# SKIRT/SKIRT9

Measured on AMD Instinct MI355X. Metric: photon packets/s (whole node), 10^6-cell octree, higher is better.
Workload: dtype f64

## Files before the change

skirt9_amd/csrc/pmc_cycle.inc:

```

    enum Event : int { EV_NONE = 0, EV_LAUNCH = 1, EV_CYCLE_DONE = 2, EV_TASK = 5, EV_DEAD = 6 };


    template<bool EMISSION = false>
    __device__ __forceinline__ int nextObserver(const DevScene& S, int slot, double rx, double ry, double rz, int g)
    {
        const SlotArrays& A = S.slots;
        while (g < S.num_instruments)
        {
            bool need = false;
            int j = g;
            do
            {
                const DevInstrument& I = S.inst[j];
                const bool seen = (I.include_sed && insideAperture(I, rx, ry, rz)) || (I.include_ifu && pixelOnDetector(I, rx, ry, rz) >= 0);
                if (seen && (EMISSION ? A.obsEll[(int64_t)j * A.num_slots + slot] : S.mono ? S.inst[j].mono_ell : A.ell[(int64_t)j * A.num_slots + slot]) >= 0)
                    need = true;
                ++j;
            } while (j < S.num_instruments && S.inst[j].same_observer);
            if (need) return g;
            g = j;
        }
        return g;
    }

    constexpr int PEEL_SORT_TILE = 2048;
    __device__ __forceinline__ uint32_t peelTile(const PeelSortArgs& ps, const DevInstrument& I, double x, double y, double z)
    {
        x -= ps.centre[0], y -= ps.centre[1], z -= ps.centre[2];
        const double xpp = -I.sinphi * x + I.cosphi * y;
        const double ypp = -I.cosphi * I.costheta * x - I.sinphi * I.costheta * y + I.sintheta * z;
        int tx = (int)(xpp * ps.scale + 0.5 * PMC_PEEL_TILES), ty = (int)(ypp * ps.scale + 0.5 * PMC_PEEL_TILES);
        tx = tx < 0 ? 0 : tx >= PMC_PEEL_TILES ? PMC_PEEL_TILES - 1 : tx;
        ty = ty < 0 ? 0 : ty >= PMC_PEEL_TILES ? PMC_PEEL_TILES - 1 : ty;
        return (uint32_t)(ty * PMC_PEEL_TILES + tx);
    }
#ifndef PMC_PROP_KEY_CONES
#define PMC_PROP_KEY_CONES 1
#endif
#ifndef PMC_PROP_KEY_BLOCKS
#define PMC_PROP_KEY_BLOCKS 1
#endif
    __device__ __forceinline__ uint32_t propSortKey(const DevScene& S, double x, double y, double z, double kx, double ky, double kz)
    {
#if PMC_PROP_KEY_CONES
        const uint32_t oct = S.grid_kind == PMC_GRID_VORONOI ? (uint32_t)(voroCone(kx, ky, kz) >> 2)
                                                             : (kx < 0. ? 1u : 0u) | (ky < 0. ? 2u : 0u) | (kz < 0. ? 4u : 0u);
#else
        const uint32_t oct = (kx < 0. ? 1u : 0u) | (ky < 0. ? 2u : 0u) | (kz < 0. ? 4u : 0u);
#endif
        constexpr int B = PMC_PROP_KEY_BLOCKS;
        int ix = (int)((x - S.gx0) / (S.gx1 - S.gx0) * B), iy = (int)((y - S.gy0) / (S.gy1 - S.gy0) * B), iz = (int)((z - S.gz0) / (S.gz1 - S.gz0) * B);
        ix = ix < 0 ? 0 : ix >= B ? B - 1 : ix;
        iy = iy < 0 ? 0 : iy >= B ? B - 1 : iy;
        iz = iz < 0 ? 0 : iz >= B ? B - 1 : iz;
        return oct * (uint32_t)(B * B * B) + (uint32_t)((iz * B + iy) * B + ix);
    }
    template<int GRID>
    __device__ __forceinline__ bool prepareWalk(const DevScene& S, const GridLds& G, Counters& cnt, int slot, int record, int mode,
                                                double rx, double ry, double rz, double kx, double ky, double kz, double target,
                                                double sext, int& hint, PeelRec* sortedOut = nullptr, bool deferScan = false)
    {
        const SlotArrays& A = S.slots;
        const TaskArrays& K = S.tasks;
        const int64_t t = (int64_t)record * A.num_slots + slot;
        Walk w;
        w.rx = rx, w.ry = ry, w.rz = rz;
        setDirection(w, kx, ky, kz);
        if (mode == MODE_PASS1) target = INFINITY;
        const bool zeroPeel = mode == MODE_PEEL && target == -INFINITY;
        if (mode == MODE_PEEL && !zeroPeel) target = nextAfterToward(target, true);
        cnt.paths += 1;
        int located;
        const bool ok = startWalk<GRID>(S, G, w, (GRID == GRID_CART) ? -1 : hint, located, GRID == GRID_VORO && deferScan);
        if ((GRID == GRID_TREE || GRID == GRID_BIN) && located >= 0) hint = located;
        if (zeroPeel || !ok)
        {
            if (record == 0)
                A.mint[slot] = -1;
            else
                A.ptau[(int64_t)(record - 1) * A.num_slots + slot] = zeroPeel ? INFINITY : 0.;
            if (GRID == GRID_TREE && sortedOut)
                reinterpret_cast<uint4*>(sortedOut)[3] = make_uint4(0u, PMC_TASK_NONE, (uint32_t)slot, 0u);
            else
                K.bits[t] = PMC_TASK_NONE;
            return false;
        }
        if (GRID == GRID_TREE && sortedOut)
        {
            const uint32_t bits = (uint32_t)mode | ((uint32_t)w.axis << 2) | (w.sgn << 4) | (w.e << 8);
            uint4* out = reinterpret_cast<uint4*>(sortedOut);
            const double2 a = make_double2(w.rx, w.ry), b = make_double2(w.rz, w.ds);
            const unsigned long long tbits = (unsigned long long)__double_as_longlong(target), P = (unsigned long long)w.P;
            out[0] = *reinterpret_cast<const uint4*>(&a);
            out[1] = *reinterpret_cast<const uint4*>(&b);
            out[2] = make_uint4((uint32_t)tbits, (uint32_t)(tbits >> 32), (uint32_t)P, (uint32_t)(P >> 32));
            out[3] = make_uint4((uint32_t)w.cell, bits, (uint32_t)slot, 0u);
            return true;
        }
        const bool moved = GRID != GRID_TREE || w.s != 0. || w.rx != rx || w.ry != ry || w.rz != rz;
        if (moved)
        {
            K.rx[t] = w.rx, K.ry[t] = w.ry, K.rz[t] = w.rz;
            if (GRID != GRID_TREE || record == 0) K.s0[t] = w.s;
        }
        if (GRID != GRID_TREE) K.kx[t] = w.kx, K.ky[t] = w.ky, K.kz[t] = w.kz;
        if (GRID == GRID_TREE) K.pidx[t] = w.P;
        K.ds[t] = w.ds;
        if (!(GRID == GRID_TREE && mode == MODE_PASS1)) K.target[t] = target;
        K.cell[t] = w.cell;
        K.bits[t] = (uint32_t)mode | ((uint32_t)w.axis << 2) | (w.sgn << 4) | ((GRID == GRID_TREE ? w.e : 0u) << 8)
                    | ((GRID == GRID_TREE && moved) ? PMC_TASK_MOVED : 0u);
        if (GRID == GRID_VORO) K.cijk[t] = w.ci;
        return true;
    }

    template<bool DIPOLE = false, bool EMISSION = false>
    __device__ __forceinline__ void announceCycle(const DevScene& S, int slot, uint64_t seed, Rng& rng, double rx, double ry, double rz, double kinx,
                                                  double kiny, double kinz, double W, double asym, int pscatt, const double* shares = nullptr,
                                                  const double* asyms = nullptr, const DevSource* emitter = nullptr)
    {
        const SlotArrays& A = S.slots;
        const int64_t NS = A.num_slots;
        uint32_t pmask = 0;
        int g = nextObserver<EMISSION>(S, slot, rx, ry, rz, 0);
        for (int i = 0; i < S.num_instruments; ++i)
        {
            if (i != g) continue;
            const DevInstrument& I = S.inst[i];
            double pW = W;
            if (pscatt != 0 && shares)
            {
                const double costheta = kinx * I.kx + kiny * I.ky + kinz * I.kz;
                double sum = 0.;
                for (int h = 0; h < S.num_media; ++h)
                    if (shares[h] > 0.)
                    {
                        const double value = phaseValue<DIPOLE>(S, h, asyms[h], costheta);
                        sum += value * shares[h];
                    }
                pW = W * sum;
            }
            else if (pscatt != 0)
                pW = W * scatteringPeelFactor<DIPOLE>(S, asym, kinx, kiny, kinz, I);
            else if (emitter)
                pW = W * angularProbability(*emitter, I.kx, I.ky, I.kz);
            A.ppW[(int64_t)i * NS + slot] = pW;
            pmask |= 1u << i;
            int j = i + 1;
            while (j < S.num_instruments && S.inst[j].same_observer) ++j;
// ... 30 lines not shown
        for (int i = 0; i <= S.num_instruments; ++i)
        {
            const bool prop = i == S.num_instruments;
            if (!prop && !((pmask >> i) & 1u))
            {
                S.tasks.bits[(int64_t)(1 + i) * NS + slot] = PMC_TASK_NONE;
                continue;
            }
            const DevInstrument& I = S.inst[prop ? 0 : i];
            double target = prop ? drawn : peelTaumax(A.ppW[(int64_t)i * NS + slot], (KIN && emission) ? A.obsLambda[(int64_t)i * NS + slot] : lambda);
            if (KIN && emission && !prop && target != -INFINITY)
            {
                const double sobs = A.obsExt[(int64_t)i * NS + slot];
                if (sobs != sext)
                {
                    if (sext == 0.) atomicAdd(S.counters + 7, 1ull);
                    target = sobs > 0. ? target * (sext / sobs) : INFINITY;
                }
            }
            PeelRec* place = nullptr;
            const bool deferScan = GRID == GRID_VORO && ps
                                   && (prop ? ((S.voro_defer_scan & 2) != 0 && ps->propIndex >= 0)
                                            : ((S.voro_defer_scan & 1) != 0 && ps->sortIndex[i] >= 0 && S.vobs_of_inst[i] >= 0));
            if (ps && !prop)
            {
                const int k = ps->sortIndex[i];
                if (k >= 0)
                {
                    const uint32_t at = atomicAdd(&cursors[(uint32_t)k * ps->numParts + peelTile(*ps, I, rx, ry, rz)], 1u);
                    if (at >= ps->cap)
                        atomicAdd(S.counters + 7, 1ull);
                    else if (GRID == GRID_TREE)
                        place = ps->out[k] + at;
                    else
                        ps->listOut[k][at] = slot;
                }
            }
            if (GRID != GRID_TREE && ps && prop && ps->propIndex >= 0)
            {
                const uint32_t at = atomicAdd(&cursors[(uint32_t)ps->propIndex * ps->numParts + propSortKey(S, rx, ry, rz, kx, ky, kz)], 1u);
                if (at >= ps->cap)
                    atomicAdd(S.counters + 7, 1ull);
                else
                    ps->listOut[ps->propIndex][at] = slot;
            }
            const bool exists = prepareWalk<GRID>(S, G, cnt, slot, prop ? 0 : 1 + i, prop ? (S.force_scattering ? MODE_PASS1 : MODE_PASS2) : MODE_PEEL,
                                                  rx, ry, rz, prop ? kx : I.kx, prop ? ky : I.ky, prop ? kz : I.kz, target, sext, hint,
                                                  place, deferScan);
            if (exists) made |= prop ? 1u : 2u << i;
        }
        return made;
    }

    template<int GRID, bool KIN = false>
    __global__ __launch_bounds__(256, PMC_CYCLE_MIN_WAVES) void cycleStartKernel(const int sceneSlot, const int slotBase, const int numSlots,
                                                                                 const int listCounter, int* const listOut,
                                                                                 const int* const listIn, const int listLen, const PeelSortArgs ps)
    {
        const DevScene& S = c_scene[sceneSlot];
        extern __shared__ double lds[];
        const int tid = threadIdx.x;
        const int lane = tid & 63;
        if (GRID == GRID_TREE) requireLdsBaseZero(lds);
        stageGrid<GRID>(S, lds, tid, blockDim.x);
        __syncthreads();
        const GridLds G = makeGridLds(S, lds);
        const SlotArrays& A = S.slots;
        Counters cnt = {0, 0, 0, 0, 0};
        const int slotEnd = slotBase + numSlots;
        const bool sparse = GRID == GRID_TREE && listIn != nullptr;
        if (ps.numObs > 0 && !sparse)
        {
            uint32_t* const cur = reinterpret_cast<uint32_t*>(reinterpret_cast<char*>(lds) + ps.ldsOffset);
            const int numLists = ps.numObs + (ps.propIndex >= 0 ? 1 : 0);
            for (int k = 0; k < numLists; ++k)
                for (uint32_t p = tid; p < ps.numParts; p += blockDim.x)
                    cur[(uint32_t)k * ps.numParts + p] = (uint32_t)ps.start[k][p] + ps.matrix[k][(size_t)blockIdx.x * ps.numParts + p];
            __syncthreads();
            const int tiles = (numSlots + PEEL_SORT_TILE - 1) / PEEL_SORT_TILE;
            for (int t = blockIdx.x; t < tiles; t += gridDim.x)
                for (int i = t * PEEL_SORT_TILE + tid; i < (t + 1) * PEEL_SORT_TILE && i < numSlots; i += blockDim.x)
                {
                    const int slot = slotBase + i;
                    const int md = A.mode[slot];
                    if (md & MODE_ALIVE) startCycleWalks<GRID, KIN>(S, G, cnt, slot, md, &ps, cur);
                }
        }
        else
        {
            const int end = sparse ? listLen : numSlots;
            for (int i0 = blockIdx.x * blockDim.x; i0 < end; i0 += gridDim.x * blockDim.x)
            {
                const int i = i0 + tid;
                const int slot = sparse ? (i < listLen ? listIn[i] : -1) : slotBase + i;
                const int md = (slot >= 0 && slot < slotEnd) ? A.mode[slot] : 0;
                if (md & MODE_ALIVE) startCycleWalks<GRID, KIN>(S, G, cnt, slot, md);
                if (GRID == GRID_TREE && listCounter >= 0)
                {
                    const unsigned long long m = __ballot((md & MODE_ALIVE) != 0);
                    if (m)
                    {
                        unsigned long long at = 0;
                        if (lane == __ffsll((long long)m) - 1) at = atomicAdd(S.counters + listCounter, (unsigned long long)__popcll(m));
                        at = __shfl(at, __ffsll((long long)m) - 1, 64);
                        if (md & MODE_ALIVE) listOut[(int)at + __popcll(m & ((1ull << lane) - 1ull))] = slot;
                    }
                }
            }
        }
        const unsigned long long v = waveSum(cnt.paths);
        if (lane == 0 && v) atomicAdd(S.counters + 1, v);
    }

    __global__ __launch_bounds__(256) void peelSortCountKernel(const int sceneSlot, const int slotBase, const int numSlots, const PeelSortArgs ps)
    {
        const DevScene& S = c_scene[sceneSlot];
        const SlotArrays& A = S.slots;
        __shared__ uint32_t h[PMC_SORT_OBS * PMC_PEEL_TILES * PMC_PEEL_TILES];
        const int tid = threadIdx.x;
        const int numLists = ps.numObs + (ps.propIndex >= 0 ? 1 : 0);
        for (uint32_t p = tid; p < (uint32_t)numLists * ps.numParts; p += blockDim.x) h[p] = 0u;
        __syncthreads();
        const int tiles = (numSlots + PEEL_SORT_TILE - 1) / PEEL_SORT_TILE;
        for (int t = blockIdx.x; t < tiles; t += gridDim.x)
            for (int i = t * PEEL_SORT_TILE + tid; i < (t + 1) * PEEL_SORT_TILE && i < numSlots; i += blockDim.x)
            {
                const int slot = slotBase + i;
                const int md = A.mode[slot];
                if (!(md & MODE_ALIVE)) continue;
                const double x = A.rx[slot], y = A.ry[slot], z = A.rz[slot];
                for (int k = 0; k < ps.numObs; ++k)
                    if (((uint32_t)md >> (8 + ps.obs[k])) & 1u) atomicAdd(&h[(uint32_t)k * ps.numParts + peelTile(ps, S.inst[ps.obs[k]], x, y, z)], 1u);
                if (ps.propIndex >= 0)
                    atomicAdd(&h[(uint32_t)ps.propIndex * ps.numParts + propSortKey(S, x, y, z, A.kx[slot], A.ky[slot], A.kz[slot])], 1u);
            }
        __syncthreads();
        for (int k = 0; k < numLists; ++k)
            for (uint32_t p = tid; p < ps.numParts; p += blockDim.x) ps.matrix[k][(size_t)blockIdx.x * ps.numParts + p] = h[(uint32_t)k * ps.numParts + p];
    }
    __global__ __launch_bounds__(256) void peelSortOffsetsKernel(uint32_t* __restrict__ matrix, const uint32_t groups, const uint32_t numParts,
                                                                 unsigned long long* __restrict__ totals)
    {
        __shared__ uint32_t part[16][17];
        const uint32_t pl = threadIdx.x & 15u, run = threadIdx.x >> 4;
        const uint32_t p = blockIdx.x * 16u + pl;
        const uint32_t rows = (groups + 15u) / 16u;
        const uint32_t b0 = run * rows, b1 = b0 + rows < groups ? b0 + rows : groups;
        uint32_t sum = 0u;
        if (p < numParts)
            for (uint32_t b = b0; b < b1; ++b) sum += matrix[(size_t)b * numParts + p];
        part[run][pl] = sum;
        __syncthreads();
        uint32_t before = 0u, all = 0u;
        for (uint32_t r = 0; r < 16u; ++r)
        {
            const uint32_t v = part[r][pl];
            if (r < run) before += v;
            all += v;
        }
        if (p < numParts)
        {
            for (uint32_t b = b0; b < b1; ++b)
            {
                const uint32_t c = matrix[(size_t)b * numParts + p];
// ... 7 lines not shown
```

skirt9_amd/csrc/pmc_device.h:

```cpp
#ifndef PMC_DEVICE_H
#define PMC_DEVICE_H

#include "../../include/pmc.h"
#include <stdint.h>

#define PMC_MAX_INSTRUMENTS 16
#define PMC_MAX_CONTEXTS 6
#define PMC_MAX_LEVEL 20
#define PMC_STAT_CAP 48
#define PMC_STAT_EMISSION_BIN 0x20000000
#define PMC_STAT_POOL_EXHAUSTED 0x40000000

#define PMC_LINK_NONE 0x7FFFFFFFu
#define PMC_LINK_NODE 0x80000000u
#define PMC_LINK_OCTET 0x40000000u
#define PMC_LINK_EXP_BITS 5
#define PMC_LINK_EXP_MASK 31u
#define PMC_LINK_INDEX_MASK 0x1FFFFFFu
#define PMC_LINK_MAX_INDEX ((1u << 25) - 2u)

struct CellRec
{
    double   density;
    uint32_t link[6];
// ... 273 lines not shown
    int32_t kin;
    DevVelocity vel[PMC_MAX_SOURCES];
    const BinCellRec* bin_cells;
    const BinNodeRec* bin_nodes;
    int32_t bin_root;
};

struct RfLogArgs
{
    uint32_t* keys;
    double* vals;
    unsigned long long cap;
    int32_t cursor;
    uint32_t padKey;
};
struct StatLogArgs
{
    uint32_t* keys;
    double* vals;
    unsigned long long cap;
    int cursor;
    unsigned long long* waveBase;
    uint32_t* waveFill;
    uint32_t* chunkFill;
};
#define PMC_STAT_NO_CHUNK 0xFFFFFFFFu
#define PMC_STAT_LOG_WAVES 16384
#define PMC_STAT_BUCKET_BITS 11

struct PeelRec
{
    double rx, ry, rz;
    double ds;
    double target;
    uint64_t pidx;
    uint32_t cell, bits;
    int32_t slot;
    uint32_t pad;
};
#define PMC_SORT_OBS 4
struct PeelSortArgs
{
    int32_t numObs;
    int32_t propIndex;
    int32_t obs[PMC_SORT_OBS];
    int8_t sortIndex[16];
    PeelRec* out[PMC_SORT_OBS];
    int32_t* listOut[PMC_SORT_OBS];
    uint32_t* matrix[PMC_SORT_OBS];
    const unsigned long long* start[PMC_SORT_OBS];
    uint32_t numParts;
    uint32_t cap;
    int32_t ldsOffset;
    double centre[3];
    double scale;
};
struct WalkStreamArgs
{
    int32_t numLists;
    int32_t rec[PMC_SORT_OBS];
    const int32_t* list[PMC_SORT_OBS];
    const unsigned long long* count[PMC_SORT_OBS];
    unsigned long long* xcdCursor;
    const int32_t* propList;
    const unsigned long long* propCount;
};
struct PeelSortedArgs
{
    const PeelRec* rec;
    const unsigned long long* count;
    unsigned long long* xcdCursor;
};
#ifndef PMC_PEEL_TILES
#define PMC_PEEL_TILES 32
#endif
#define PMC_VORO_RUN_UNIT_BITS 27
#define PMC_VORO_RUN_UNIT_MASK 0x07FFFFFFu
#define PMC_VORO_RUN_COUNT_UNKNOWN 31u
#define PMC_VORO_FIRST_SCAN (-1000)
#define PMC_VORO_RUN_PAD 16
#ifndef PMC_VORO_RUN_LANES
#define PMC_VORO_RUN_LANES 2
#endif
#ifndef PMC_VORO_CONES
#define PMC_VORO_CONES 192
#endif
#define PMC_RAY_STEP_CAP 100000

#define PMC_RF_LOG_CHUNK 4096
#define PMC_RF_BUCKET_BITS 13
#define PMC_RF_SHORT_RUN 4096
#define PMC_STAT_SHORT_RUN 1024

#define PMC_NUM_COUNTERS 512
#define PMC_CTR_HISTORY 8
#define PMC_CTR_WALKWORK 16
#define PMC_CTR_LIVE(g) (35 + 4 * (g))
#define PMC_CTR_TASK(g, k) (256 + 32 * (g) + (k))
#define PMC_CTR_TASKS_PER_GROUP 32
#define PMC_CTR_LIST(g) PMC_CTR_TASK(g, 30)
#define PMC_CTR_RFLOG(g) PMC_CTR_TASK(g, 31)
#define PMC_CTR_STATLOG(g) (56 + (g))
#define PMC_CTR_HBASE(g) (120 + (g))
#define PMC_CTR_HLIMIT(g) (124 + (g))
#define PMC_MAX_GROUPS 4
#define PMC_CTR_STATFREE(g) (48 + (g))
// ... 4 lines not shown
```

skirt9_amd/csrc/pmc_kernels.hip:

```cpp

#include "pmc_device.h"
#include "../../include/pmc_philox.h"
#include "../../include/pmc_tuning.h"
#include <hip/hip_runtime.h>
#include <cstdlib>
#include <cstring>
#include <float.h>
#include <math.h>
#include <algorithm>
#include <mutex>
#include <array>
#include <type_traits>
#include <utility>

#ifndef PMC_WALK_REFILL
    #define PMC_WALK_REFILL 40
#endif
#ifndef PMC_PEEL_REFILL
    #define PMC_PEEL_REFILL 32
#endif
#ifndef PMC_PROP_REFILL
    #define PMC_PROP_REFILL 40
#endif
#ifndef PMC_PEEL_BLOCK
// ... 246 lines not shown
static const auto launchKernels = flavourTable<PMC_LAUNCH_FLAVOURS>([](auto f) {
    constexpr int F = decltype(f)::value;
    return KernelFlavour<LaunchKernel>{launchKernel<F>, 0};
});
typedef void (*TraceKernel)(int, double, double, double, double, double, double, const double*, int32_t*, double*, int32_t, int32_t*);
static const auto traceKernels = flavourTable<7>([](auto f) {
    constexpr int F = decltype(f)::value;
    return KernelFlavour<TraceKernel>{traceRayKernel<RAY_GRIDS[F % 5], F % 5 == 1, (F < 5)>, 0};
});

template<typename Table> static hipError_t raiseLdsLimits(const Table& table, size_t walkMax)
{
    for (const auto& k : table)
    {
        const size_t lds = k.extraLds ? std::min(walkMax + k.extraLds, size_t(160) * 1024) : walkMax;
        hipError_t e = hipFuncSetAttribute(reinterpret_cast<const void*>(k.kernel), hipFuncAttributeMaxDynamicSharedMemorySize, (int)lds);
        if (e != hipSuccess) return e;
    }
    return hipSuccess;
}

extern "C" hipError_t pmcConfigureKernels(size_t walkLds, size_t transitionLds)
{
    static std::mutex lock;
    std::lock_guard<std::mutex> guard(lock);
    static size_t walkMax = 0, transitionMax = 0;
    walkMax = std::max(walkMax, walkLds);
    transitionMax = std::max(transitionMax, transitionLds);
    {
        hipError_t e = hipFuncSetAttribute(reinterpret_cast<const void*>(&rfReduceKernel), hipFuncAttributeMaxDynamicSharedMemorySize,
                                           (int)(sizeof(double) << PMC_RF_BUCKET_BITS));
        if (e != hipSuccess) return e;
        const int scatterLds = (int)(size_t(RF_TILE) * (sizeof(double) + sizeof(uint32_t)) + size_t(2) * RF_MAX_PARTS * sizeof(uint32_t));
        e = hipFuncSetAttribute(reinterpret_cast<const void*>(&rfScatterKernel<PMC_RF_BUCKET_BITS>), hipFuncAttributeMaxDynamicSharedMemorySize, scatterLds);
        if (e != hipSuccess) return e;
        e = hipFuncSetAttribute(reinterpret_cast<const void*>(&rfScatterKernel<PMC_STAT_BUCKET_BITS>), hipFuncAttributeMaxDynamicSharedMemorySize, scatterLds);
        if (e != hipSuccess) return e;
        e = hipFuncSetAttribute(reinterpret_cast<const void*>(&statReduceKernel), hipFuncAttributeMaxDynamicSharedMemorySize,
                                (int)(5 * sizeof(double) << PMC_STAT_BUCKET_BITS));
        if (e != hipSuccess) return e;
    }
    for (hipError_t e : {raiseLdsLimits(peelKernels, walkMax), raiseLdsLimits(peel2Kernels, walkMax), raiseLdsLimits(propKernels, walkMax),
                         raiseLdsLimits(walkKernels, walkMax), raiseLdsLimits(binWalkKernels, walkMax), raiseLdsLimits(traceKernels, walkMax),
                         raiseLdsLimits(integrateKernels, walkMax), raiseLdsLimits(integrateWeightedKernels, walkMax), raiseLdsLimits(locateKernels, walkMax)})
        if (e != hipSuccess) return e;
    const struct
    {
        const void* kernel;
        size_t lds;
    } all[] = {{reinterpret_cast<const void*>(&transitionKernel), transitionMax},
               {reinterpret_cast<const void*>(&transitionDipoleKernel), transitionMax},
               {reinterpret_cast<const void*>(&transitionKinKernel), transitionMax},
               {reinterpret_cast<const void*>(&transitionKinDipoleKernel), transitionMax},
               {reinterpret_cast<const void*>(&cycleStartKernel<GRID_TREE, true>), walkMax + 16 + size_t(PMC_SORT_OBS) * PMC_PEEL_TILES * PMC_PEEL_TILES * sizeof(uint32_t)},
               {reinterpret_cast<const void*>(&cycleStartKernel<GRID_CART, true>), walkMax + 16 + size_t(PMC_SORT_OBS) * PMC_PEEL_TILES * PMC_PEEL_TILES * sizeof(uint32_t)},
               {reinterpret_cast<const void*>(&cycleStartKernel<GRID_VORO, true>), walkMax + 16 + size_t(PMC_SORT_OBS) * PMC_PEEL_TILES * PMC_PEEL_TILES * sizeof(uint32_t)},
               {reinterpret_cast<const void*>(&cycleStartKernel<GRID_TREE>), walkMax + 16 + size_t(PMC_SORT_OBS) * PMC_PEEL_TILES * PMC_PEEL_TILES * sizeof(uint32_t)},
               {reinterpret_cast<const void*>(&cycleStartKernel<GRID_CART>), walkMax + 16 + size_t(PMC_SORT_OBS) * PMC_PEEL_TILES * PMC_PEEL_TILES * sizeof(uint32_t)},
               {reinterpret_cast<const void*>(&cycleStartKernel<GRID_VORO>), walkMax + 16 + size_t(PMC_SORT_OBS) * PMC_PEEL_TILES * PMC_PEEL_TILES * sizeof(uint32_t)},
               {reinterpret_cast<const void*>(&cycleStartKernel<GRID_BIN, true>), walkMax + 16 + size_t(PMC_SORT_OBS) * PMC_PEEL_TILES * PMC_PEEL_TILES * sizeof(uint32_t)},
               {reinterpret_cast<const void*>(&cycleStartKernel<GRID_BIN>), walkMax + 16 + size_t(PMC_SORT_OBS) * PMC_PEEL_TILES * PMC_PEEL_TILES * sizeof(uint32_t)}};
    for (const auto& k : all)
    {
        hipError_t e = hipFuncSetAttribute(k.kernel, hipFuncAttributeMaxDynamicSharedMemorySize, (int)k.lds);
        if (e != hipSuccess) return e;
    }
    return raiseLdsLimits(launchKernels, transitionMax);
}

extern "C" int pmcPropHasCheckpoints(int flavour, size_t ldsBytes)
{
    return flavourHasCheckpointRoom(flavour) && !pmcTune("PMC_PROP_NO_CHECKPOINTS") && ((ldsBytes + 15) & ~size_t(15)) + PROP_CKPT_BYTES <= size_t(160) * 1024;
}
extern "C" int pmcPeelHasQueues(int form, size_t ldsBytes)
{
    return (form & 2) == 0 && ((ldsBytes + 15) & ~size_t(15)) + pmcPeelQueueBytes() <= size_t(160) * 1024;
}

extern "C" int pmcWalkBlocksPerCU(int gridKind, int kind, int wide, int block, size_t ldsBytes)
{
    const void* kernel;
    if (gridKind == PMC_GRID_OCTREE && kind == 1)
        kernel = reinterpret_cast<const void*>(peelKernels[wide ? 1 : 0].kernel);
    else if (gridKind == PMC_GRID_OCTREE)
    {
        if (pmcPropHasCheckpoints(0, ldsBytes)) ldsBytes = ((ldsBytes + 15) & ~size_t(15)) + PROP_CKPT_BYTES;
        kernel = reinterpret_cast<const void*>(propKernels[wide ? 8 : 0].kernel);
    }
    else if (gridKind == PMC_GRID_BINTREE)
        kernel = reinterpret_cast<const void*>(binWalkKernels[0].kernel);
    else
        kernel = reinterpret_cast<const void*>(walkKernels[gridKind == PMC_GRID_VORONOI ? 8 : 0].kernel);
    int n = 0;
    return hipOccupancyMaxActiveBlocksPerMultiprocessor(&n, kernel, block, ldsBytes) == hipSuccess ? n : 0;
}

extern "C" int pmcPeelBlock(void)
{
    return PMC_PEEL_BLOCK;
}
extern "C" int pmcPropBlock(void)
{
    return PMC_PROP_BLOCK;
}


extern "C" hipError_t pmcLaunchWalk(int slot, int gridKind, int flavour, int taskBase, int numTaskRecords, int taskCounter,
                                    uint64_t seed, int grid, int block, size_t ldsBytes, const WalkStreamArgs* tasks, hipStream_t stream)
{
    WalkStreamArgs ws;
// ... 132 lines not shown
    out->max_parts = RF_MAX_PARTS;
    out->reduce_span = (int64_t)PMC_RF_REDUCE_SPAN;
    out->rf_short_run = PMC_RF_SHORT_RUN;
    out->stat_short_run = PMC_STAT_SHORT_RUN;
}
extern "C" hipError_t pmcLaunchLogPartition(int stat, const uint32_t* keys, const double* vals, uint32_t* sortedKeys, double* sortedVals, unsigned long long n,
                                            int numParts, void* temp, int numCU, const uint32_t* fills, hipStream_t stream)
{
    return stat ? launchPartition<PMC_STAT_BUCKET_BITS>(keys, vals, sortedKeys, sortedVals, n, numParts, temp, numCU, stream, fills)
                : launchPartition<PMC_RF_BUCKET_BITS>(keys, vals, sortedKeys, sortedVals, n, numParts, temp, numCU, stream, fills);
}
extern "C" hipError_t pmcLaunchStatMerge(int slot, int blocks, hipStream_t stream)
{
    hipLaunchKernelGGL(statMergeKernel, dim3(blocks), dim3(256), 0, stream, slot);
    return hipGetLastError();
}

extern "C" hipError_t pmcLaunchTransition(int slot, int flavour, int slotBase, int numSlots, int group, uint64_t seed, const int* list, int listLen, int maxBlocks,
                                          size_t ldsBytes, const StatLogArgs* statLog, uint64_t count, hipStream_t stream)
{
    const StatLogArgs none = {nullptr, nullptr, 0ull, 0, nullptr, nullptr, nullptr};
    const int block = PMC_TRANSITION_BLOCK;
    const int grid = std::max(1, std::min(((list ? listLen : numSlots) + block - 1) / block, maxBlocks));
    const auto kernel = (flavour & 2) ? ((flavour & 1) ? transitionKinDipoleKernel : transitionKinKernel) : ((flavour & 1) ? transitionDipoleKernel : transitionKernel);
    hipLaunchKernelGGL(kernel, dim3(grid), dim3(block), ldsBytes, stream, slot, slotBase, numSlots, group, seed, list, listLen,
                       statLog ? *statLog : none);
    hipError_t e = hipGetLastError();
    if (e != hipSuccess || list) return e;
    hipLaunchKernelGGL(endedScanKernel, dim3(1), dim3(PMC_SCAN_THREADS), 0, stream, slot, slotBase, numSlots, group, (unsigned long long)count);
    return hipGetLastError();
}

extern "C" hipError_t pmcLaunchLaunch(int slot, int flavour, int slotBase, int numSlots, int group, uint64_t first, uint64_t count, uint64_t seed, int initial,
                                      int maxBlocks, size_t ldsBytes, const StatLogArgs* statLog, hipStream_t stream)
{
    const StatLogArgs none = {nullptr, nullptr, 0ull, 0, nullptr, nullptr, nullptr};
    const int grid = std::max(1, std::min((numSlots + 255) / 256, maxBlocks));
    if (flavour < 0 || flavour >= PMC_LAUNCH_FLAVOURS) return hipErrorInvalidValue;
    hipLaunchKernelGGL(launchKernels[flavour].kernel, dim3(grid), dim3(256), ldsBytes, stream, slot, slotBase, numSlots, group, first, count, seed, initial,
                       statLog ? *statLog : none);
    return hipGetLastError();
}

extern "C" hipError_t pmcLaunchCycleStart(int slot, int gridKind, int kin, int slotBase, int numSlots, int listCounter, int* listOut, const int* listIn,
                                          int listLen, int maxBlocks, size_t ldsBytes, const PeelSortArgs* sort, hipStream_t stream)
{
    PeelSortArgs ps;
    std::memset(&ps, 0, sizeof(ps));
    if (sort) ps = *sort;
    if (ps.numObs > 0)
    {
        ps.ldsOffset = int((ldsBytes + 15) & ~size_t(15));
        ldsBytes = size_t(ps.ldsOffset) + size_t(ps.numObs + (ps.propIndex >= 0 ? 1 : 0)) * PEEL_SORT_PARTS * sizeof(uint32_t);
    }
    const int grid = std::max(1, std::min(((listIn ? listLen : numSlots) + 255) / 256, maxBlocks));
    const auto kernel = kin ? (gridKind == PMC_GRID_OCTREE ? cycleStartKernel<GRID_TREE, true> : gridKind == PMC_GRID_VORONOI ? cycleStartKernel<GRID_VORO, true>
                               : gridKind == PMC_GRID_BINTREE ? cycleStartKernel<GRID_BIN, true> : cycleStartKernel<GRID_CART, true>)
                            : (gridKind == PMC_GRID_OCTREE ? cycleStartKernel<GRID_TREE> : gridKind == PMC_GRID_VORONOI ? cycleStartKernel<GRID_VORO>
                               : gridKind == PMC_GRID_BINTREE ? cycleStartKernel<GRID_BIN> : cycleStartKernel<GRID_CART>);
    hipLaunchKernelGGL(kernel, dim3(grid), dim3(256), ldsBytes, stream, slot, slotBase, numSlots, listCounter, listOut, listIn, listLen, ps);
    return hipGetLastError();
}

namespace
{
    __global__ __launch_bounds__(256) void dipoleCosineKernel(const double* __restrict__ u, const int64_t n, double* __restrict__ out)
    {
        const int64_t i = (int64_t)blockIdx.x * blockDim.x + threadIdx.x;
        if (i < n) out[i] = PhaseDipole::cosineFor(u[i]);
    }
}
extern "C" hipError_t pmcLaunchDipoleCosines(const double* u, int64_t n, double* out, hipStream_t stream)
{
    if (n <= 0) return hipSuccess;
    hipLaunchKernelGGL(dipoleCosineKernel, dim3((unsigned)((n + 255) / 256)), dim3(256), 0, stream, u, n, out);
    return hipGetLastError();
}

namespace
{
    __global__ __launch_bounds__(256) void sourceVelocityKernel(const int sceneSlot, const int source, const double* __restrict__ r, const int64_t n,
                                                                double* __restrict__ out)
    {
        const int64_t i = (int64_t)blockIdx.x * blockDim.x + threadIdx.x;
        if (i >= n) return;
        double vx, vy, vz;
        sourceVelocity(c_scene[sceneSlot].vel[source], r[3 * i], r[3 * i + 1], r[3 * i + 2], vx, vy, vz);
        out[3 * i] = vx, out[3 * i + 1] = vy, out[3 * i + 2] = vz;
    }
}
extern "C" hipError_t pmcLaunchSourceVelocities(int slot, int source, const double* r, int64_t n, double* out, hipStream_t stream)
{
    if (n <= 0) return hipSuccess;
    hipLaunchKernelGGL(sourceVelocityKernel, dim3((unsigned)((n + 255) / 256)), dim3(256), 0, stream, slot, source, r, n, out);
    return hipGetLastError();
}

namespace
{
    __global__ __launch_bounds__(256) void deviceFunctionKernel(const int sceneSlot, const int function, const double* __restrict__ args, const int widthIn,
                                                                const int64_t n, double* __restrict__ out, const int widthOut)
    {
        const int64_t i = (int64_t)blockIdx.x * blockDim.x + threadIdx.x;
        if (i >= n) return;
        const double* a = args + i * widthIn;
        double* o = out + i * widthOut;
        switch (function)
// ... 114 lines not shown
```

skirt9_amd/csrc/pmc_walk.inc:

```

    struct Walk
    {
        double rx, ry, rz;
        double kx, ky, kz;
        double ikx, iky, ikz;
        double tau, s;
        double ds;
        double dens;
        uint32_t e;
        uint64_t P;
        int ci, cj, ck;
        int cell;
        int axis;
        int lastm;
        uint32_t sgn;
    };

    struct GridLds
    {
        const double* grid;
        const char* gtab;
        uint32_t stride;
        uint32_t fieldBits;
    };
// ... 117 lines not shown
        while ((int32_t)link < 0)
        {
            const int bit = (int)(link & PMC_LINK_EXP_MASK) - 1;
            const int l = ((ix >> bit) & 1) | (((iy >> bit) & 1) << 1) | (((iz >> bit) & 1) << 2);
            link = S.nodes[(link >> PMC_LINK_EXP_BITS) & PMC_LINK_INDEX_MASK].child[l];
        }
        return link == PMC_LINK_NONE ? -1 : (int)(link >> PMC_LINK_EXP_BITS);
    }
    __device__ __forceinline__ bool leafContains(const DevScene& S, const GridLds& L, int m, double x, double y, double z)
    {
        uint32_t ox, oy, oz, szb;
        decodeBox(S.leaves[m].code, L.stride, ox, oy, oz, szb);
        return x >= tabAt(L.gtab, ox) && x <= tabAt(L.gtab, ox + szb) && y >= tabAt(L.gtab, oy) && y <= tabAt(L.gtab, oy + szb)
               && z >= tabAt(L.gtab, oz) && z <= tabAt(L.gtab, oz + szb);
    }
    __device__ __forceinline__ int listNeighbor(const DevScene& S, const GridLds& L, int m, int wall, double x, double y, double z)
    {
        int b = S.nbr_start[6 * (int64_t)m + wall], e = S.nbr_start[6 * (int64_t)m + wall + 1];
        for (int q = b; q < e; ++q)
        {
            int cand = S.nbr_list[q];
            if (leafContains(S, L, cand, x, y, z)) return cand;
        }
        return -1;
    }

    template<bool CHECK>
    __device__ __forceinline__ bool treeEnter(const char* leaves, const GridLds& L, Walk& w, int m)
    {
        const uint4 h = *reinterpret_cast<const uint4*>(leaves + ((uint32_t)m << 4));
        uint32_t ox, oy, oz, e;
        decodeBoxWords(h.x, h.y, L.stride, ox, oy, oz, e);
        const uint32_t szb = 8u << e;
        const double X0 = tabAt(L.gtab, ox), X1 = tabAt(L.gtab, ox + szb);
        const double Y0 = tabAt(L.gtab, oy), Y1 = tabAt(L.gtab, oy + szb);
        const double Z0 = tabAt(L.gtab, oz), Z1 = tabAt(L.gtab, oz + szb);
        const double rx = w.rx, ry = w.ry, rz = w.rz;
        if (CHECK)
        {
            const bool inside = rx > X0 && rx < X1 && ry > Y0 && ry < Y1 && rz > Z0 && rz < Z1;
            if (!inside) return false;
        }
        const bool nx = w.kx < 0.0, ny = w.ky < 0.0, nz = w.kz < 0.0;
        double ds;
        int ax;
        exitDistance<false>(w, nx ? X0 : X1, ny ? Y0 : Y1, nz ? Z0 : Z1, ds, ax);
        w.ds = ds;
        w.axis = ax;
        w.e = e;
        w.P = (uint64_t)(ox >> 3) | ((uint64_t)((oy - L.stride) >> 3) << L.fieldBits) | ((uint64_t)((oz - 2u * L.stride) >> 3) << (2u * L.fieldBits));
        w.cell = m;
        w.dens = __longlong_as_double(((long long)h.w << 32) | h.z);
        return true;
    }

    enum LaneState : int
    {
        ST_ACTIVE = 0,
        ST_HIT = 1,
        ST_SLOW = 2,
        ST_EXIT = 3,
        ST_IDLE = 4,
        ST_EDGE = 5,
        ST_FIRST = 6
    };

    struct TreeConst
    {
        double gx0, gy0, gz0;
        double gx1, gy1, gz1;
        double sx8, sy8, sz8;
        double bx8, by8, bz8;
        uint32_t stride;
        const char* gtab;
        const char* cellTab;
        uint32_t numCells;
    };

    __device__ __forceinline__ bool treeStepSlow(const DevScene& S, const GridLds& L, Walk& w)
    {
        const int old = w.cell;
        const int wall = 2 * w.axis + (((w.sgn >> w.axis) & 1u) ? 0 : 1);
        int next = listNeighbor(S, L, old, wall, w.rx, w.ry, w.rz);
        if (next < 0) next = topDown(S, L, w.rx, w.ry, w.rz);
        if (next == old)
        {
            w.rx = nextAfterToward(w.rx, w.kx < 0.);
            w.ry = nextAfterToward(w.ry, w.ky < 0.);
            w.rz = nextAfterToward(w.rz, w.kz < 0.);
            next = topDown(S, L, w.rx, w.ry, w.rz);
        }
        if (next < 0 || next == old) return false;
        treeEnter<false>(reinterpret_cast<const char*>(S.leaves), L, w, next);
        return true;
    }


    __device__ __forceinline__ void cartEnter(const DevScene& S, const GridLds& L, Walk& w)
    {
        const double* xv = L.grid;
        const double* yv = L.grid + (S.nx + 1);
        const double* zv = yv + (S.ny + 1);
        const int m = w.ck + S.nz * w.cj + S.nz * S.ny * w.ci;
        const double xE = (w.kx < 0.0) ? xv[w.ci] : xv[w.ci + 1];
        const double yE = (w.ky < 0.0) ? yv[w.cj] : yv[w.cj + 1];
        const double zE = (w.kz < 0.0) ? zv[w.ck] : zv[w.ck + 1];
// ... 696 lines not shown
```

Baseline: 212.3 million.

## Add fast octree cycle-start path reusing hinted leaf box for all walks

```diff
diff --git a/skirt9_amd/csrc/pmc_cycle.inc b/skirt9_amd/csrc/pmc_cycle.inc
--- a/skirt9_amd/csrc/pmc_cycle.inc
+++ b/skirt9_amd/csrc/pmc_cycle.inc
@@ -25,6 +25,7 @@
     }
 
     constexpr int PEEL_SORT_TILE = 2048;
+    constexpr size_t CYCLE_SLOW_LIST_BYTES = PEEL_SORT_TILE * sizeof(uint16_t) + 16;
     __device__ __forceinline__ uint32_t peelTile(const PeelSortArgs& ps, const DevInstrument& I, double x, double y, double z)
     {
         x -= ps.centre[0], y -= ps.centre[1], z -= ps.centre[2];
@@ -55,6 +56,17 @@
         iy = iy < 0 ? 0 : iy >= B ? B - 1 : iy;
         iz = iz < 0 ? 0 : iz >= B ? B - 1 : iz;
         return oct * (uint32_t)(B * B * B) + (uint32_t)((iz * B + iy) * B + ix);
+    }
+    __device__ __forceinline__ void storeSortedWalkStart(const Walk& w, int slot, int mode, double target, PeelRec* sortedOut)
+    {
+        const uint32_t bits = (uint32_t)mode | ((uint32_t)w.axis << 2) | (w.sgn << 4) | (w.e << 8);
+        uint4* out = reinterpret_cast<uint4*>(sortedOut);
+        const double2 a = make_double2(w.rx, w.ry), b = make_double2(w.rz, w.ds);
+        const unsigned long long tbits = (unsigned long long)__double_as_longlong(target), P = (unsigned long long)w.P;
+        out[0] = *reinterpret_cast<const uint4*>(&a);
+        out[1] = *reinterpret_cast<const uint4*>(&b);
+        out[2] = make_uint4((uint32_t)tbits, (uint32_t)(tbits >> 32), (uint32_t)P, (uint32_t)(P >> 32));
+        out[3] = make_uint4((uint32_t)w.cell, bits, (uint32_t)slot, 0u);
     }
     template<int GRID>
     __device__ __forceinline__ bool prepareWalk(const DevScene& S, const GridLds& G, Counters& cnt, int slot, int record, int mode,
@@ -88,14 +100,7 @@
         }
         if (GRID == GRID_TREE && sortedOut)
         {
-            const uint32_t bits = (uint32_t)mode | ((uint32_t)w.axis << 2) | (w.sgn << 4) | (w.e << 8);
-            uint4* out = reinterpret_cast<uint4*>(sortedOut);
-            const double2 a = make_double2(w.rx, w.ry), b = make_double2(w.rz, w.ds);
-            const unsigned long long tbits = (unsigned long long)__double_as_longlong(target), P = (unsigned long long)w.P;
-            out[0] = *reinterpret_cast<const uint4*>(&a);
-            out[1] = *reinterpret_cast<const uint4*>(&b);
-            out[2] = make_uint4((uint32_t)tbits, (uint32_t)(tbits >> 32), (uint32_t)P, (uint32_t)(P >> 32));
-            out[3] = make_uint4((uint32_t)w.cell, bits, (uint32_t)slot, 0u);
+            storeSortedWalkStart(w, slot, mode, target, sortedOut);
             return true;
         }
         const bool moved = GRID != GRID_TREE || w.s != 0. || w.rx != rx || w.ry != ry || w.rz != rz;
@@ -232,6 +237,137 @@
         return made;
     }
 
+    template<bool KIN>
+    __device__ __forceinline__ bool startCycleFast(const DevScene& S, const GridLds& G, Counters& cnt, int slot, int modeWord, const PeelSortArgs* ps = nullptr,
+                                                   uint32_t* cursors = nullptr)
+    {
+        const SlotArrays& A = S.slots;
+        const int64_t NS = A.num_slots;
+        const uint32_t pmask = ((uint32_t)modeWord >> 8) & 0xFFFFu;
+        const int hint = A.mint[slot];
+        const double rx = A.rx[slot], ry = A.ry[slot], rz = A.rz[slot];
+        const double kx = A.kx[slot], ky = A.ky[slot], kz = A.kz[slot];
+        const double lambda = S.mono ? S.mono_lambda : A.lambda[slot];
+        const double drawn = S.force_scattering ? 0. : A.tausample[slot];
+        const bool emission = KIN && A.nscatt[slot] == 0;
+        double pw[4];
+        uint32_t rest = pmask;
+#pragma unroll
+        for (int q = 0; q < 4; ++q)
+        {
+            pw[q] = rest ? A.ppW[(int64_t)(__ffs((int)rest) - 1) * NS + slot] : 1.;
+            rest &= rest - 1u;
+        }
+        if (hint < 0 || emission) return false;
+        const LeafBox B = leafBox(reinterpret_cast<const char*>(S.leaves), G, hint);
+        bool fast = strictlyInside(B, rx, ry, rz) && rx > S.gx0 && rx < S.gx1 && ry > S.gy0 && ry < S.gy1 && rz > S.gz0 && rz < S.gz1;
+#pragma unroll
+        for (int q = 0; q < 4; ++q) fast = fast && !(q < __popc(pmask) && pw[q] / lambda <= 0.);
+        for (; fast && rest; rest &= rest - 1u) fast = !(A.ppW[(int64_t)(__ffs((int)rest) - 1) * NS + slot] / lambda <= 0.);
+        if (!fast) return false;
+        Walk w;
+        w.rx = rx, w.ry = ry, w.rz = rz;
+        w.s = 0.;
+#pragma unroll 1
+        for (int i = 0; i <= S.num_instruments; ++i)
+        {
+            const bool prop = i == S.num_instruments;
+            if (!prop && !((pmask >> i) & 1u))
+            {
+                S.tasks.bits[(int64_t)(1 + i) * NS + slot] = PMC_TASK_NONE;
+                continue;
+            }
+            const DevInstrument& I = S.inst[prop ? 0 : i];
+            const int mode = prop ? (S.force_scattering ? MODE_PASS1 : MODE_PASS2) : MODE_PEEL;
+            double target = drawn;
+            if (mode == MODE_PASS1) target = INFINITY;
+            if (!prop)
+            {
+                const int q = __popc(pmask & ((1u << i) - 1u));
+                const double pW = q == 0 ? pw[0] : q == 1 ? pw[1] : q == 2 ? pw[2] : q == 3 ? pw[3] : A.ppW[(int64_t)i * NS + slot];
+                target = nextAfterToward(peelTaumax(pW, lambda), true);
+            }
+            PeelRec* place = nullptr;
+            if (ps && !prop)
+            {
+                const int k = ps->sortIndex[i];
+                if (k >= 0)
+                {
+                    const uint32_t at = atomicAdd(&cursors[(uint32_t)k * ps->numParts + peelTile(*ps, I, rx, ry, rz)], 1u);
+                    if (at >= ps->cap)
+                        atomicAdd(S.counters + 7, 1ull);
+                    else
+                        place = ps->out[k] + at;
+                }
+            }
+            setDirection(w, prop ? kx : I.kx, prop ? ky : I.ky, prop ? kz : I.kz);
+            enterLeafBox(B, w, hint);
+            cnt.paths += 1;
+            if (place)
+                storeSortedWalkStart(w, slot, mode, target, place);
+            else
+            {
+                const TaskArrays& K = S.tasks;
+                const int64_t t = (int64_t)(prop ? 0 : 1 + i) * NS + slot;
+                K.pidx[t] = w.P;
+                K.ds[t] = w.ds;
+                if (mode != MODE_PASS1) K.target[t] = target;
+                K.cell[t] = w.cell;
+                K.bits[t] = (uint32_t)mode | ((uint32_t)w.axis << 2) | (w.sgn << 4) | (w.e << 8);
+            }
+        }
+        return true;
+    }
+
+    __device__ __forceinline__ uint32_t bitsBelowLane(unsigned long long m)
+    {
+        return __builtin_amdgcn_mbcnt_hi((uint32_t)(m >> 32), __builtin_amdgcn_mbcnt_lo((uint32_t)m, 0u));
+    }
+    template<bool KIN>
+    __device__ __forceinline__ void startTreeTile(const DevScene& S, const GridLds& G, Counters& cnt, int firstSlot, int n, const PeelSortArgs& ps,
+                                                  uint32_t* cursors, uint16_t* slow, uint32_t* words, int turn)
+    {
+        const SlotArrays& A = S.slots;
+        const int tid = threadIdx.x;
+        uint32_t* const count = words + turn;
+        uint32_t* const hinted = words + 2 + turn;
+        bool twoPasses = false;
+        int todo = n;
+        if (!ps.plainStart)
+        {
+            if (tid < n && (A.mode[firstSlot + tid] & MODE_ALIVE) && A.mint[firstSlot + tid] >= 0) *hinted = 1u;
+            __syncthreads();
+            twoPasses = *hinted != 0u;
+            if (tid == 0) words[turn ^ 1] = 0u, words[2 + (turn ^ 1)] = 0u;
+        }
+        if (twoPasses)
+        {
+            for (int i0 = 0; i0 < n; i0 += blockDim.x)
+            {
+                const int i = i0 + tid;
+                const int md = i < n ? A.mode[firstSlot + i] : 0;
+                const bool left = (md & MODE_ALIVE) && !startCycleFast<KIN>(S, G, cnt, firstSlot + i, md, &ps, cursors);
+                const unsigned long long m = __ballot(left);
+                if (m)
+                {
+                    const uint32_t rank = bitsBelowLane(m);
+                    uint32_t at = 0u;
+                    if (left && rank == 0u) at = atomicAdd(count, (uint32_t)__popcll(m));
+                    at = __shfl(at, __ffsll((long long)m) - 1, 64);
+                    if (left) slow[at + rank] = (uint16_t)i;
+                }
+            }
+        }
+        if (!ps.plainStart) __syncthreads();
+        if (twoPasses) todo = (int)*count;
+        for (int j = tid; j < todo; j += blockDim.x)
+        {
+            const int slot = firstSlot + (twoPasses ? (int)slow[j] : j);
+            const int md = A.mode[slot];
+            if (md & MODE_ALIVE) startCycleWalks<GRID_TREE, KIN>(S, G, cnt, slot, md, &ps, cursors);
+        }
+    }
+
     template<int GRID, bool KIN = false>
     __global__ __launch_bounds__(256, PMC_CYCLE_MIN_WAVES) void cycleStartKernel(const int sceneSlot, const int slotBase, const int numSlots,
                                                                                  const int listCounter, int* const listOut,
@@ -256,15 +392,26 @@
             for (int k = 0; k < numLists; ++k)
                 for (uint32_t p = tid; p < ps.numParts; p += blockDim.x)
                     cur[(uint32_t)k * ps.numParts + p] = (uint32_t)ps.start[k][p] + ps.matrix[k][(size_t)blockIdx.x * ps.numParts + p];
+            uint16_t* const slow = reinterpret_cast<uint16_t*>(cur + (uint32_t)numLists * ps.numParts);
+            uint32_t* const words = reinterpret_cast<uint32_t*>(slow + PEEL_SORT_TILE);
+            if (GRID == GRID_TREE && tid < 4) words[tid] = 0u;
             __syncthreads();
             const int tiles = (numSlots + PEEL_SORT_TILE - 1) / PEEL_SORT_TILE;
-            for (int t = blockIdx.x; t < tiles; t += gridDim.x)
-                for (int i = t * PEEL_SORT_TILE + tid; i < (t + 1) * PEEL_SORT_TILE && i < numSlots; i += blockDim.x)
-                {
-                    const int slot = slotBase + i;
-                    const int md = A.mode[slot];
-                    if (md & MODE_ALIVE) startCycleWalks<GRID, KIN>(S, G, cnt, slot, md, &ps, cur);
-                }
+            if (GRID == GRID_TREE)
+            {
+                int turn = 0;
+                for (int t = blockIdx.x; t < tiles; t += gridDim.x, turn ^= 1)
+                    startTreeTile<KIN>(S, G, cnt, slotBase + t * PEEL_SORT_TILE, min(PEEL_SORT_TILE, numSlots - t * PEEL_SORT_TILE), ps, cur, slow, words,
+                                       turn);
+            }
+            else
+                for (int t = blockIdx.x; t < tiles; t += gridDim.x)
+                    for (int i = t * PEEL_SORT_TILE + tid; i < (t + 1) * PEEL_SORT_TILE && i < numSlots; i += blockDim.x)
+                    {
+                        const int slot = slotBase + i;
+                        const int md = A.mode[slot];
+                        if (md & MODE_ALIVE) startCycleWalks<GRID, KIN>(S, G, cnt, slot, md, &ps, cur);
+                    }
         }
         else
         {
@@ -274,7 +421,8 @@
                 const int i = i0 + tid;
                 const int slot = sparse ? (i < listLen ? listIn[i] : -1) : slotBase + i;
                 const int md = (slot >= 0 && slot < slotEnd) ? A.mode[slot] : 0;
-                if (md & MODE_ALIVE) startCycleWalks<GRID, KIN>(S, G, cnt, slot, md);
+                if ((md & MODE_ALIVE) && (GRID != GRID_TREE || ps.plainStart || !startCycleFast<KIN>(S, G, cnt, slot, md)))
+                    startCycleWalks<GRID, KIN>(S, G, cnt, slot, md);
                 if (GRID == GRID_TREE && listCounter >= 0)
                 {
                     const unsigned long long m = __ballot((md & MODE_ALIVE) != 0);
@@ -289,7 +437,7 @@
             }
         }
         const unsigned long long v = waveSum(cnt.paths);
-        if (lane == 0 && v) atomicAdd(S.counters + 1, v);
+        if ((GRID == GRID_TREE ? bitsBelowLane(~0ull) == 0u : lane == 0) && v) atomicAdd(S.counters + 1, v);
     }
 
     __global__ __launch_bounds__(256) void peelSortCountKernel(const int sceneSlot, const int slotBase, const int numSlots, const PeelSortArgs ps)
diff --git a/skirt9_amd/csrc/pmc_device.h b/skirt9_amd/csrc/pmc_device.h
--- a/skirt9_amd/csrc/pmc_device.h
+++ b/skirt9_amd/csrc/pmc_device.h
@@ -349,6 +349,7 @@
     uint32_t numParts;
     uint32_t cap;
     int32_t ldsOffset;
+    int32_t plainStart;
     double centre[3];
     double scale;
 };
diff --git a/skirt9_amd/csrc/pmc_kernels.hip b/skirt9_amd/csrc/pmc_kernels.hip
--- a/skirt9_amd/csrc/pmc_kernels.hip
+++ b/skirt9_amd/csrc/pmc_kernels.hip
@@ -322,10 +322,10 @@
                {reinterpret_cast<const void*>(&transitionDipoleKernel), transitionMax},
                {reinterpret_cast<const void*>(&transitionKinKernel), transitionMax},
                {reinterpret_cast<const void*>(&transitionKinDipoleKernel), transitionMax},
-               {reinterpret_cast<const void*>(&cycleStartKernel<GRID_TREE, true>), walkMax + 16 + size_t(PMC_SORT_OBS) * PMC_PEEL_TILES * PMC_PEEL_TILES * sizeof(uint32_t)},
+               {reinterpret_cast<const void*>(&cycleStartKernel<GRID_TREE, true>), walkMax + 16 + size_t(PMC_SORT_OBS) * PMC_PEEL_TILES * PMC_PEEL_TILES * sizeof(uint32_t) + CYCLE_SLOW_LIST_BYTES},
                {reinterpret_cast<const void*>(&cycleStartKernel<GRID_CART, true>), walkMax + 16 + size_t(PMC_SORT_OBS) * PMC_PEEL_TILES * PMC_PEEL_TILES * sizeof(uint32_t)},
                {reinterpret_cast<const void*>(&cycleStartKernel<GRID_VORO, true>), walkMax + 16 + size_t(PMC_SORT_OBS) * PMC_PEEL_TILES * PMC_PEEL_TILES * sizeof(uint32_t)},
-               {reinterpret_cast<const void*>(&cycleStartKernel<GRID_TREE>), walkMax + 16 + size_t(PMC_SORT_OBS) * PMC_PEEL_TILES * PMC_PEEL_TILES * sizeof(uint32_t)},
+               {reinterpret_cast<const void*>(&cycleStartKernel<GRID_TREE>), walkMax + 16 + size_t(PMC_SORT_OBS) * PMC_PEEL_TILES * PMC_PEEL_TILES * sizeof(uint32_t) + CYCLE_SLOW_LIST_BYTES},
                {reinterpret_cast<const void*>(&cycleStartKernel<GRID_CART>), walkMax + 16 + size_t(PMC_SORT_OBS) * PMC_PEEL_TILES * PMC_PEEL_TILES * sizeof(uint32_t)},
                {reinterpret_cast<const void*>(&cycleStartKernel<GRID_VORO>), walkMax + 16 + size_t(PMC_SORT_OBS) * PMC_PEEL_TILES * PMC_PEEL_TILES * sizeof(uint32_t)},
                {reinterpret_cast<const void*>(&cycleStartKernel<GRID_BIN, true>), walkMax + 16 + size_t(PMC_SORT_OBS) * PMC_PEEL_TILES * PMC_PEEL_TILES * sizeof(uint32_t)},
@@ -564,7 +564,9 @@
     {
         ps.ldsOffset = int((ldsBytes + 15) & ~size_t(15));
         ldsBytes = size_t(ps.ldsOffset) + size_t(ps.numObs + (ps.propIndex >= 0 ? 1 : 0)) * PEEL_SORT_PARTS * sizeof(uint32_t);
-    }
+        if (gridKind == PMC_GRID_OCTREE) ldsBytes += CYCLE_SLOW_LIST_BYTES;
+    }
+    ps.plainStart = pmcTune("PMC_CYCLE_START_PLAIN") != nullptr;
     const int grid = std::max(1, std::min(((listIn ? listLen : numSlots) + 255) / 256, maxBlocks));
     const auto kernel = kin ? (gridKind == PMC_GRID_OCTREE ? cycleStartKernel<GRID_TREE, true> : gridKind == PMC_GRID_VORONOI ? cycleStartKernel<GRID_VORO, true>
                                : gridKind == PMC_GRID_BINTREE ? cycleStartKernel<GRID_BIN, true> : cycleStartKernel<GRID_CART, true>)
diff --git a/skirt9_amd/csrc/pmc_walk.inc b/skirt9_amd/csrc/pmc_walk.inc
--- a/skirt9_amd/csrc/pmc_walk.inc
+++ b/skirt9_amd/csrc/pmc_walk.inc
@@ -193,6 +193,43 @@
         w.cell = m;
         w.dens = __longlong_as_double(((long long)h.w << 32) | h.z);
         return true;
+    }
+
+    struct LeafBox
+    {
+        double X0, X1, Y0, Y1, Z0, Z1;
+        uint64_t P;
+        uint32_t e;
+    };
+    __device__ __forceinline__ LeafBox leafBox(const char* leaves, const GridLds& L, int m)
+    {
+        const uint2 h = *reinterpret_cast<const uint2*>(leaves + ((uint32_t)m << 4));
+        uint32_t ox, oy, oz, e;
+        decodeBoxWords(h.x, h.y, L.stride, ox, oy, oz, e);
+        const uint32_t szb = 8u << e;
+        LeafBox B;
+        B.X0 = tabAt(L.gtab, ox), B.X1 = tabAt(L.gtab, ox + szb);
+        B.Y0 = tabAt(L.gtab, oy), B.Y1 = tabAt(L.gtab, oy + szb);
+        B.Z0 = tabAt(L.gtab, oz), B.Z1 = tabAt(L.gtab, oz + szb);
+        B.e = e;
+        B.P = (uint64_t)(ox >> 3) | ((uint64_t)((oy - L.stride) >> 3) << L.fieldBits) | ((uint64_t)((oz - 2u * L.stride) >> 3) << (2u * L.fieldBits));
+        return B;
+    }
+    __device__ __forceinline__ bool strictlyInside(const LeafBox& B, double rx, double ry, double rz)
+    {
+        return rx > B.X0 && rx < B.X1 && ry > B.Y0 && ry < B.Y1 && rz > B.Z0 && rz < B.Z1;
+    }
+    __device__ __forceinline__ void enterLeafBox(const LeafBox& B, Walk& w, int m)
+    {
+        const bool nx = w.kx < 0.0, ny = w.ky < 0.0, nz = w.kz < 0.0;
+        double ds;
+        int ax;
+        exitDistance<false>(w, nx ? B.X0 : B.X1, ny ? B.Y0 : B.Y1, nz ? B.Z0 : B.Z1, ds, ax);
+        w.ds = ds;
+        w.axis = ax;
+        w.e = B.e;
+        w.P = B.P;
+        w.cell = m;
     }
 
     enum LaneState : int
```

Result: no change. 213.5 million (median of 6 runs) (+0.6%).
